# huggingface/parler-tts

Hardware: NVIDIA H100
Metric: audio codec tokens/sec (all codebooks) (higher is better)
Workload: dtype bf16

## Files before the change

include/ptts_b200.h:

```cpp
#ifndef PTTS_B200_H
#define PTTS_B200_H

#include <stdint.h>

#ifdef __cplusplus
extern "C" {
#endif

#define PTTS_OK 0
#define PTTS_EINVAL 1
#define PTTS_ECUDA 2
#define PTTS_ESTATE 3

#define PTTS_BF16 0
#define PTTS_F32 1
#define PTTS_I64 2
#define PTTS_I32 3

#define PTTS_HEAD_DIM 64

typedef struct ptts_decoder_config {
  int32_t hidden_size;
  int32_t num_layers;
  int32_t num_heads;
// ... 190 lines not shown

int ptts_dac_blob_bytes(const ptts_dac_config* cfg, int64_t* out_bytes);
int ptts_dac_num_tensors(const ptts_dac_config* cfg, int32_t* out);
int ptts_dac_pack(const ptts_dac_config* cfg, void* blob, int32_t name_id, const void* src,
                  int32_t src_dtype, int64_t numel, void* stream);
int ptts_dac_workspace_bytes(const ptts_dac_config* cfg, int32_t B, int32_t T, int64_t* out_bytes);
int ptts_dac_decode(const ptts_dac_config* cfg, const void* blob, void* workspace, int64_t workspace_bytes,
                    const int64_t* codes, int32_t B, int32_t T, void* audio_out, void* stream);
int ptts_dac_decode2(const ptts_dac_config* cfg, const void* blob, void* workspace, int64_t workspace_bytes,
                     const int64_t* codes, int32_t B, int32_t T, const int32_t* frame_lengths, void* audio_out,
                     void* stream);
int ptts_dac_decode3(const ptts_dac_config* cfg, const void* blob, void* workspace, int64_t workspace_bytes,
                     const int64_t* codes, int32_t B, int32_t T_codes, int32_t T,
                     const int32_t* frame_start, const int32_t* frame_lengths,
                     const int32_t* emit_lo, const int32_t* emit_hi, void* audio_out, void* stream);

int ptts_dac_encoder_blob_bytes(const ptts_dac_config* cfg, int64_t* out_bytes);
int ptts_dac_encoder_num_tensors(const ptts_dac_config* cfg, int32_t* out);
int ptts_dac_encoder_pack(const ptts_dac_config* cfg, void* enc_blob, int32_t name_id, const void* src,
                          int32_t src_dtype, int64_t numel, void* stream);
int ptts_dac_encode_workspace_bytes(const ptts_dac_config* cfg, int32_t B, int32_t samples, int64_t* out_bytes);
int ptts_dac_encode(const ptts_dac_config* cfg, const void* dec_blob, const void* enc_blob, void* workspace,
                    int64_t workspace_bytes, const void* audio, int32_t B, int32_t samples, int32_t n_q, int64_t* codes_out,
                    void* latents_out, void* stream);
int ptts_dac_encode2(const ptts_dac_config* cfg, const void* dec_blob, const void* enc_blob, void* workspace,
                     int64_t workspace_bytes, const void* audio, int32_t B, int32_t samples, const int32_t* sample_lengths,
                     int32_t n_q, int64_t* codes_out, void* latents_out, void* stream);

int ptts_op_dac_conv(int32_t dtype, int32_t kernel, int32_t kind, int32_t B, int32_t Cin, int32_t Cout, int32_t T, int32_t taps,
                     int32_t dil_or_stride, int32_t samples, const void* weight, const void* bias, const void* alpha,
                     const void* alpha_next, const void* x, const void* res, void* out_raw, void* out_act, int32_t tanh_out,
                     const int32_t* frame_lengths, int32_t frames, void* scratch, void* stream);

#ifdef __cplusplus
}
#endif
#endif
```

parler_tts_b200/_lib.py:

```python
from __future__ import annotations
import ctypes as C
import os

import torch

_HERE = os.path.dirname(os.path.abspath(__file__))
LIB_PATH = os.environ.get("PTTS_LIB") or os.path.join(_HERE, "csrc", "libptts_b200.so")

BF16, F32, I64, I32 = 0, 1, 2, 3
OK, EINVAL, ECUDA, ESTATE = 0, 1, 2, 3


class DecoderConfigC(C.Structure):
    _fields_ = [(n, C.c_int32) for n in (
        "hidden_size", "num_layers", "num_heads", "num_kv_heads", "num_cross_kv_heads", "ffn_dim", "vocab_size",
        "num_codebooks", "max_positions", "rope", "activation", "dtype", "bos_token_id", "pad_token_id",
        "eos_token_id")] + [("rope_theta", C.c_float), ("layer_norm_eps", C.c_float)]


class GenParamsC(C.Structure):
    _fields_ = [("max_length", C.c_int32), ("min_new_tokens", C.c_int32), ("do_sample", C.c_int32),
                ("top_k", C.c_int32), ("top_p", C.c_float), ("temperature", C.c_float), ("seed", C.c_uint64),
                ("suppress_special", C.c_int32), ("codebook_size", C.c_int32),
                ("row_base", C.c_int32), ("input_len", C.c_int32)]
# ... 61 lines not shown
    "ptts_session_logits": (C.c_int, [_VP, C.POINTER(_VP)]),
    "ptts_session_scores": (C.c_int, [_VP, C.POINTER(_VP)]),
    "ptts_session_raw_ids": (C.c_int, [_VP, C.POINTER(_VP), C.POINTER(_I32)]),
    "ptts_session_state": (C.c_int, [_VP, C.POINTER(_VP)]),
    "ptts_session_eos_seen": (C.c_int, [_VP, C.POINTER(_VP)]),
    "ptts_session_launches": (C.c_int, [_VP, C.POINTER(_I64)]),
    "ptts_session_fused": (C.c_int, [_VP, C.POINTER(_I32)]),
    "ptts_session_set_profile": (C.c_int, [_VP, _VP]),
    "ptts_delay_build": (C.c_int, [_VP, _I32, _I32, _I32, _I64, _I64, _I32, _VP, _VP]),
    "ptts_delay_apply": (C.c_int, [_VP, _I32, _I32, _I64, _VP, _I64, _VP, _VP]),
    "ptts_logits_processor": (C.c_int, [_VP, _I32, _I32, _I64, _VP, _I32, _I64, _I32, _VP, _VP]),
    "ptts_op_sample_phase": (C.c_int, [_VP, _I32, _VP]),
    "ptts_op_linear": (C.c_int, [C.POINTER(DecoderConfigC), _VP, _I32, _I32, _VP, _I32, _I32, _I32, _VP, _VP, _VP]),
    "ptts_op_linear2": (C.c_int, [C.POINTER(DecoderConfigC), _VP, _I32, _I32, _VP, _I32, _I32, _I32, _VP, _VP, _I32, _VP, _VP]),
    "ptts_op_attention": (C.c_int, [_I32, _I32, _I32, _I32, _I32, _I32, _I32, _I32, _I32, _I32, _VP, _VP, _VP, _VP, _VP, _VP,
                                    _I32, _I32, _VP, _VP]),
    "ptts_op_attention_probs": (C.c_int, [_I32, _I32, _I32, _I32, _I32, _I32, _I32, _I32, _I32, _I32, _VP, _VP, _VP, _I64, _VP,
                                          _VP, _I32, _VP, _VP]),
    "ptts_dac_blob_bytes": (C.c_int, [C.POINTER(DacConfigC), C.POINTER(_I64)]),
    "ptts_dac_num_tensors": (C.c_int, [C.POINTER(DacConfigC), C.POINTER(_I32)]),
    "ptts_dac_pack": (C.c_int, [C.POINTER(DacConfigC), _VP, _I32, _VP, _I32, _I64, _VP]),
    "ptts_dac_workspace_bytes": (C.c_int, [C.POINTER(DacConfigC), _I32, _I32, C.POINTER(_I64)]),
    "ptts_dac_decode": (C.c_int, [C.POINTER(DacConfigC), _VP, _VP, _I64, _VP, _I32, _I32, _VP, _VP]),
    "ptts_dac_decode2": (C.c_int, [C.POINTER(DacConfigC), _VP, _VP, _I64, _VP, _I32, _I32, _VP, _VP, _VP]),
    "ptts_dac_decode3": (C.c_int, [C.POINTER(DacConfigC), _VP, _VP, _I64, _VP, _I32, _I32, _I32, _VP, _VP, _VP, _VP, _VP, _VP]),
    "ptts_dac_encoder_blob_bytes": (C.c_int, [C.POINTER(DacConfigC), C.POINTER(_I64)]),
    "ptts_dac_encoder_num_tensors": (C.c_int, [C.POINTER(DacConfigC), C.POINTER(_I32)]),
    "ptts_dac_encoder_pack": (C.c_int, [C.POINTER(DacConfigC), _VP, _I32, _VP, _I32, _I64, _VP]),
    "ptts_dac_encode_workspace_bytes": (C.c_int, [C.POINTER(DacConfigC), _I32, _I32, C.POINTER(_I64)]),
    "ptts_dac_encode": (C.c_int, [C.POINTER(DacConfigC), _VP, _VP, _VP, _I64, _VP, _I32, _I32, _I32, _VP, _VP, _VP]),
    "ptts_dac_encode2": (C.c_int, [C.POINTER(DacConfigC), _VP, _VP, _VP, _I64, _VP, _I32, _I32, _VP, _I32, _VP, _VP, _VP]),
    "ptts_op_dac_conv": (C.c_int, [_I32, _I32, _I32, _I32, _I32, _I32, _I32, _I32, _I32, _I32, _VP, _VP, _VP, _VP, _VP, _VP, _VP,
                                   _VP, _I32, _VP, _I32, _VP, _VP]),
}
EXPORTED_SYMBOLS = tuple(_SIGS)

_lib = None


def lib():
    global _lib
    if _lib is None:
        if not os.path.exists(LIB_PATH):
            raise ImportError(
                f"{LIB_PATH} is missing: build it with `python parler_tts_b200/csrc/build.py` "
                "(or __graft_entry__.build()).  parler_tts_b200 has no CPU / PyTorch fallback.")
        l = C.CDLL(LIB_PATH)
        for name, (res, args) in _SIGS.items():
            fn = getattr(l, name)
            fn.restype, fn.argtypes = res, args
        _lib = l
    return _lib


def check(code: int):
    if code == OK:
        return
    msg = lib().ptts_last_error().decode("utf-8", "replace")
    if code == EINVAL:
        raise ValueError(msg)
    raise RuntimeError(msg)


def dtype_code(dt: torch.dtype) -> int:
    if dt == torch.bfloat16:
        return BF16
# ... 22 lines not shown
```

parler_tts_b200/csrc/api.cu:

```cuda
#include <cstdarg>
#include <cstdlib>
#include <cstring>
#include <new>
#include <vector>

#include "common.cuh"
#include "dac.h"
#include "kernels.h"
#include "layout.h"
#include "step.h"

namespace ptts {
static thread_local std::string g_err;
void set_error(const std::string& m) { g_err = m; }
int fail(int code, const char* fmt, ...) {
  char buf[1024];
  va_list ap;
  va_start(ap, fmt);
  vsnprintf(buf, sizeof(buf), fmt, ap);
  va_end(ap);
  g_err = buf;
  return code;
}
static bool env_flag(const char* name, bool dflt) {
// ... 1212 lines not shown
        a.alpha = tiled;
      }
      a.out = out_raw; a.tanh_out = tanh_out ? 1 : 0;
      return launch_conv(a, dtype, B, st, ragged(a));
    }
    case 1: {
      PTTS_REQUIRE(conv_tc_supported(a.Cin, a.Cout), "op_dac_conv: conv_tc_kernel does not take Cin %d, Cout %d", a.Cin, a.Cout);
      PTTS_REQUIRE(!alpha && !tanh_out && samples == 0, "op_dac_conv: conv_tc_kernel has no input snake, tanh or samples");
      PTTS_REQUIRE(!out_act == !alpha_next, "op_dac_conv: out_act and alpha_next go together");
      if (kind == 2) {
        if (int e = pack_strided_conv(weight, dtype, scratch, PTTS_BF16, Cout, Cin, s, 1, st)) return e;
      } else if (int e = pack_conv_kmajor(weight, dtype, scratch, kind == 1 ? Cin : Cout, kind == 1 ? Cout : Cin, k_src, kind == 1, st)) {
        return e;
      }
      return launch_conv_tc(a, scratch, a.n_taps * a.n_phase, alpha_next, out_raw, out_act, B, st, ragged(a));
    }
    case 2: {
      PTTS_REQUIRE(kind == 0 && Cout == 1 && taps == 7 && dil_or_stride == 1 && final_conv_supported(Cin),
                   "op_dac_conv: the final conv is conv_same(C, 1, T, 7, 1) with final_conv_supported(C), got Cin %d Cout %d taps %d", Cin, Cout, taps);
      PTTS_REQUIRE(!alpha && !alpha_next && !res && !out_act && out_raw && tanh_out && samples == 0, "op_dac_conv: the final conv writes tanh to out_raw only");
      if (int e = pack_conv(weight, dtype, scratch, dtype, Cout, Cin, 7, 0, st)) return e;
      return launch_final_conv_tanh(x, scratch, bias, out_raw, Cin, T, B, frame_lengths, frames, st);
    }
    default: {
      PTTS_REQUIRE(kind == 0 && Cin == 1 && taps == 7 && dil_or_stride == 1 && samples > 0 && samples <= T,
                   "op_dac_conv: the input conv is conv_same(1, C, T, 7, 1) over 1..T samples");
      PTTS_REQUIRE(!alpha && !res && !tanh_out && !frame_lengths && alpha_next && out_raw && out_act, "op_dac_conv: the input conv writes raw and snake_{alpha_next}");
      if (int e = pack_conv(weight, dtype, scratch, dtype, Cout, 1, 7, 0, st)) return e;
      return launch_enc_input_conv(x, scratch, bias, alpha_next, out_raw, out_act, Cout, samples, T, B, nullptr, 0, st);
    }
  }
}

}
```

parler_tts_b200/csrc/attention.cu:

```cuda
#include "common.cuh"
#include "kernels.h"
#include "attn_core.cuh"

namespace ptts {

template <typename T>
__global__ void __launch_bounds__(ATT_THREADS) attention_kernel(AttnArgs p) {
  extern __shared__ __align__(16) float sm[];
  pdl_launch_dependents();
  pdl_wait();
  if (p.ctrl != nullptr && p.ctrl->active == 0) return;
  const int per = (p.q_len + (int)gridDim.z - 1) / (int)gridDim.z;
  attention_item<T>(p, blockIdx.y, blockIdx.x, sm, threadIdx.x, [] { __syncthreads(); }, (int)blockIdx.z * per, (int)(blockIdx.z + 1) * per);
}

template <typename T, bool RAGGED>
__global__ void __launch_bounds__(256) attention_decode_kernel(AttnArgs p) {
  extern __shared__ __align__(128) unsigned char smd[];
  const int warp = threadIdx.x >> 5, lane = threadIdx.x & 31;
  uint64_t* bars = reinterpret_cast<uint64_t*>(smd) + 2 * warp;
  unsigned char* sm_warp = smd + 128 + (size_t)warp * attn_decode_smem_per_warp<T>();
  attention_decode_init_warp(bars, lane);
  pdl_launch_dependents();
  pdl_wait();
  if (p.ctrl != nullptr && p.ctrl->active == 0) return;
  const int pair = warp >> 1, part = warp & 1;
  const int it = blockIdx.x * 4 + pair;
  if (it >= p.B * p.nkv) return;
  int past = p.past_len;
  if (p.past_from_ctrl) past = p.prefix + p.ctrl->cur_len - 1 - (RAGGED ? row_shift(p.shift, it / p.nkv) : 0);
  uint32_t parity = 0;
  float* xch = reinterpret_cast<float*>(smd + 128 + (size_t)8 * attn_decode_smem_per_warp<T>()) + pair * 128;
  attention_decode_item_warp<T>(p, it / p.nkv, it % p.nkv, past, sm_warp, bars, lane, parity, part, 2, xch, pair + 1);
}

constexpr int PRE_TC_WARPS = 8;
constexpr int PRE_TC_WARP_BYTES = 2 * ATT_TC_STAGE_BYTES + 768;
__global__ void __launch_bounds__(PRE_TC_WARPS * 32) attention_prefill_tc_kernel(AttnArgs p) {
  extern __shared__ __align__(128) unsigned char smp[];
  const int warp = threadIdx.x >> 5, lane = threadIdx.x & 31;
  uint64_t* bars = reinterpret_cast<uint64_t*>(smp) + 2 * warp;
  unsigned char* ring0 = smp + 128 + (size_t)warp * PRE_TC_WARP_BYTES;
  unsigned char* ring1 = ring0 + ATT_TC_STAGE_BYTES;
  float* fbuf = reinterpret_cast<float*>(ring1 + ATT_TC_STAGE_BYTES);
  attention_decode_init_warp(bars, lane);
  pdl_launch_dependents();
  pdl_wait();
  if (p.ctrl != nullptr && p.ctrl->active == 0) return;
  const int b = blockIdx.y, h = blockIdx.x;
  const int past = p.past_len;
  const int kvb = b / p.kv_b_div;
  bf16* kc = reinterpret_cast<bf16*>(p.kcache) + (size_t)kvb * p.kv_b_stride + (size_t)h * p.kv_h_stride;
  bf16* vc = reinterpret_cast<bf16*>(p.vcache) + (size_t)kvb * p.kv_b_stride + (size_t)h * p.kv_h_stride;
  if (!p.cross) {
    const bf16* rope_cos = reinterpret_cast<const bf16*>(p.rope_cos);
    const bf16* rope_sin = reinterpret_cast<const bf16*>(p.rope_sin);
    for (int idx = threadIdx.x; idx < p.q_len * 2 * HD; idx += PRE_TC_WARPS * 32) {
      const int j = idx / (2 * HD), e = idx - j * 2 * HD, d = e & (HD - 1);
      const size_t r = (size_t)b * p.q_len + j;
      const int pos = past + j;
      if (e < HD) {
        const bf16* src = reinterpret_cast<const bf16*>(p.knew) + r * p.ldkv + p.k_col0 + h * HD;
        float x = __bfloat162float(src[d]);
        if (p.rope) {
          const float xp = __bfloat162float(src[d < HD / 2 ? d + HD / 2 : d - HD / 2]);
          x = rope_elem<bf16>(x, xp, d, rope_cos + (size_t)pos * HD, rope_sin + (size_t)pos * HD);
        }
        kc[(size_t)pos * HD + kv_swz(pos, d)] = __float2bfloat16_rn(x);
      } else {
        const bf16* src = reinterpret_cast<const bf16*>(p.vnew) + r * p.ldkv + p.v_col0 + h * HD;
        vc[(size_t)pos * HD + kv_swz(pos, d)] = src[d];
      }
    }
    __threadfence();
    asm volatile("fence.proxy.async.global;" ::: "memory");
    __syncthreads();
  }
  uint32_t parity = 0;
  for (int j = warp; j < p.q_len; j += PRE_TC_WARPS) {
    const size_t r = (size_t)b * p.q_len + j;
    TcItem it{};
    it.q = reinterpret_cast<const bf16*>(p.q) + r * p.ldq + p.q_col0 + (size_t)h * HD;
    it.knew = nullptr; it.vnew = nullptr;
    it.kc = kc; it.vc = vc;
    it.km = p.key_mask ? p.key_mask + (size_t)kvb * p.mask_ld : nullptr; it.mask_len = p.mask_len;
    it.n_cached = p.cross ? p.kv_len : past + j + 1;
    it.pos = past + j; it.cross = 1;
    it.rope = p.rope; it.rope_cos = reinterpret_cast<const bf16*>(p.rope_cos); it.rope_sin = reinterpret_cast<const bf16*>(p.rope_sin);
    it.scale = p.scale;
    it.out = reinterpret_cast<bf16*>(p.out) + r * p.ldo + (size_t)h * HD;
    attention_decode_item_warp_tc(it, ring0, ring1, fbuf, bars, lane, parity, 0, 1, nullptr, 0);
    asm volatile("fence.proxy.async.shared::cta;" ::: "memory");
    __syncwarp();
  }
}

int launch_attention(const AttnArgs& a, int dtype, cudaStream_t st, bool pdl, bool prefill_tc) {
  if (a.q_len > 1 && dtype == PTTS_BF16 && a.nh == a.nkv && a.kv_t_stride == HD && !a.past_from_ctrl && prefill_tc) {
    const size_t smem = 128 + (size_t)PRE_TC_WARPS * PRE_TC_WARP_BYTES;
    static bool attr_p = false;
    if (!attr_p) {
      PTTS_CHECK_CUDA(cudaFuncSetAttribute(attention_prefill_tc_kernel, cudaFuncAttributeMaxDynamicSharedMemorySize, (int)smem));
      attr_p = true;
    }
    cudaLaunchConfig_t cfg{};
    cfg.gridDim = dim3(a.nkv, a.B);
    cfg.blockDim = dim3(PRE_TC_WARPS * 32);
    cfg.dynamicSmemBytes = smem;
    cfg.stream = st;
    cudaLaunchAttribute at[1];
    at[0].id = cudaLaunchAttributeProgrammaticStreamSerialization;
    at[0].val.programmaticStreamSerializationAllowed = 1;
    cfg.attrs = at;
    cfg.numAttrs = pdl ? 1 : 0;
    PTTS_CHECK_CUDA(cudaLaunchKernelEx(&cfg, attention_prefill_tc_kernel, a));
    return PTTS_OK;
  }
  if (a.q_len == 1) {
    const size_t smem_d = 128 + (size_t)8 * (dtype == PTTS_BF16 ? attn_decode_smem_per_warp<bf16>() : attn_decode_smem_per_warp<float>()) + 4 * 128 * sizeof(float);
    static bool attr_d = false;
    if (!attr_d) {
      PTTS_CHECK_CUDA(cudaFuncSetAttribute(attention_decode_kernel<bf16, false>, cudaFuncAttributeMaxDynamicSharedMemorySize, 200 * 1024));
      PTTS_CHECK_CUDA(cudaFuncSetAttribute(attention_decode_kernel<float, false>, cudaFuncAttributeMaxDynamicSharedMemorySize, 200 * 1024));
      PTTS_CHECK_CUDA(cudaFuncSetAttribute(attention_decode_kernel<bf16, true>, cudaFuncAttributeMaxDynamicSharedMemorySize, 200 * 1024));
      PTTS_CHECK_CUDA(cudaFuncSetAttribute(attention_decode_kernel<float, true>, cudaFuncAttributeMaxDynamicSharedMemorySize, 200 * 1024));
      attr_d = true;
    }
    cudaLaunchConfig_t cfg{};
    cfg.gridDim = dim3((a.B * a.nkv + 3) / 4);
    cfg.blockDim = dim3(256);
    cfg.dynamicSmemBytes = smem_d;
    cfg.stream = st;
    cudaLaunchAttribute at[1];
    at[0].id = cudaLaunchAttributeProgrammaticStreamSerialization;
    at[0].val.programmaticStreamSerializationAllowed = 1;
    cfg.attrs = at;
    cfg.numAttrs = pdl ? 1 : 0;
    const bool rg = a.shift != nullptr;
    if (dtype == PTTS_BF16) PTTS_CHECK_CUDA(cudaLaunchKernelEx(&cfg, rg ? attention_decode_kernel<bf16, true> : attention_decode_kernel<bf16, false>, a));
    else PTTS_CHECK_CUDA(cudaLaunchKernelEx(&cfg, rg ? attention_decode_kernel<float, true> : attention_decode_kernel<float, false>, a));
    return PTTS_OK;
  }
  const int kv_capacity = a.kv_capacity;
  PTTS_REQUIRE(a.B > 0 && a.nkv > 0 && a.q_len > 0, "attention: empty problem");
  const size_t smem = (size_t)(HD + ATT_WARPS * HD + 8 + kv_capacity) * sizeof(float);
  PTTS_REQUIRE(smem <= 200 * 1024, "attention: kv length %d needs %zu B of shared memory (> 200 KB)", kv_capacity, smem);
  static bool attr_done = false;
// ... 24 lines not shown
```

parler_tts_b200/csrc/dac.cu:

```cuda
#include <utility>
#include <vector>

#include "common.cuh"
#include "dac.h"

namespace ptts {

template <typename T>
__device__ __forceinline__ float snake_fn(float x, float alpha, float inv) {
  const float s = DT<T>::rnd(sinf(DT<T>::rnd(alpha * x)));
  return DT<T>::rnd(x + DT<T>::rnd(inv * DT<T>::rnd(s * s)));
}

constexpr int CT_M = 64, CT_N = 64, CT_K = 16, CT_AROWS = 128, CT_MAXTAPS = 7;

template <typename T, bool SAMPLES, bool WINDOW = false>
__global__ void __launch_bounds__(256) conv_kernel(ConvArgs p, RowLengths rl) {
  __shared__ float As[CT_K][CT_AROWS];
  __shared__ __align__(16) float Bs[CT_MAXTAPS][CT_K][CT_N];
  const int tid = threadIdx.x, tx = tid & 15, ty = tid >> 4;
  const int phase = blockIdx.z % p.n_phase, b = blockIdx.z / p.n_phase;
  const int q0 = blockIdx.x * CT_M, co0 = blockIdx.y * CT_N;
  const int wt_base = p.wt_base + phase * p.wt_phase_step;
  const int off_last = p.off_base + (p.n_taps - 1) * p.off_step;
// ... 267 lines not shown
  const DacWindow* win;
  std::vector<Margin> m;
  size_t i = 1;
  RowLengths next(int up_in, int up_out) {
    RowLengths r{fl, T, up_in, up_out};
    if (win != nullptr) { r.emit_lo = win->emit_lo; r.emit_hi = win->emit_hi; r.m_lo = m[i].lo; r.m_hi = m[i].hi; }
    i++;
    return r;
  }
};

static int decode_tc(const ptts_dac_config& c, const DacLayout& L, const char* bl, const DacWorkspace& W, void* ws, int B, int T,
                     WalkRows& rows, void* audio, cudaStream_t st) {
  auto P = [&](int i) { return (const void*)(bl + L.t[i].off); };
  auto conv = [&](ConvArgs a, const void* x, int w, int b, const void* res, void* out_raw, void* out_act, const void* alpha_next) {
    a.x = x; a.bias = P(b); a.res = res;
    return launch_conv_tc(a, bl + L.t[w].off_k, a.n_taps * a.n_phase, alpha_next, out_raw, out_act, B, st, rows.next(a.Tin / T, a.Tout / T));
  };
  char* act = W.buf(ws, 0);
  char* oth = W.buf(ws, 1);
  char* res = W.buf(ws, 2);
  const int C = c.decoder_dim, nb = c.n_blocks;
  if (int e = conv(conv_same(c.latent_dim, C, T, 7, 1), W.buf(ws, 3), L.conv1_w, L.conv1_b, nullptr, nullptr, act, P(L.block[0].snake1))) return e;
  int Tl = T;
  for (int bi = 0; bi < nb; bi++) {
    const DacDecBlock& blk = L.block[bi];
    const int cout = C >> (bi + 1), s = c.strides[bi];
    if (int e = conv(conv_up(C >> bi, cout, Tl, s), act, blk.conv_t1_w, blk.conv_t1_b, nullptr, res, oth, P(blk.res[0].snake1))) return e;
    std::swap(act, oth);
    Tl *= s;
    for (int r = 0; r < 3; r++) {
      const DacResUnit& u = blk.res[r];
      const int next = r < 2 ? blk.res[r + 1].snake1 : bi + 1 < nb ? L.block[bi + 1].snake1 : L.snake1;
      if (int e = conv(conv_same(cout, cout, Tl, 7, kDilation[r]), act, u.conv1_w, u.conv1_b, nullptr, nullptr, oth, P(u.snake2))) return e;
      if (int e = conv(conv_same(cout, cout, Tl, 1, 1), oth, u.conv2_w, u.conv2_b, res, res, act, P(next))) return e;
    }
  }
  const int cl = C >> nb;
  const RowLengths rl = rows.next(Tl / T, Tl / T);
  if (final_conv_supported(cl))
    return launch_final_conv_tanh(act, P(L.conv2_w), P(L.conv2_b), audio, cl, Tl, B, rl.frame_lengths, T, st, rl.emit_lo, rl.emit_hi);
  ConvArgs f = conv_same(cl, 1, Tl, 7, 1);
  f.x = act; f.w = P(L.conv2_w); f.bias = P(L.conv2_b); f.out = audio; f.tanh_out = 1;
  return launch_conv(f, c.dtype, B, st, rl);
}

static int decode_generic(const ptts_dac_config& c, const DacLayout& L, const char* bl, const DacWorkspace& W, void* ws, int B, int T,
                          WalkRows& rows, void* audio, cudaStream_t st) {
  auto P = [&](int i) { return (const void*)(bl + L.t[i].off); };
  auto conv = [&](ConvArgs a, const void* x, const void* alpha, int w, int b, const void* res, void* out) {
    a.x = x; a.alpha = alpha; a.w = P(w); a.bias = P(b); a.res = res; a.out = out;
    return launch_conv(a, c.dtype, B, st, rows.next(a.Tin / T, a.Tout / T));
  };
  char* cur = W.buf(ws, 0);
  char* oth = W.buf(ws, 1);
  const int C = c.decoder_dim;
  if (int e = conv(conv_same(c.latent_dim, C, T, 7, 1), W.buf(ws, 3), nullptr, L.conv1_w, L.conv1_b, nullptr, cur)) return e;
  int Tl = T;
  for (int bi = 0; bi < c.n_blocks; bi++) {
    const DacDecBlock& blk = L.block[bi];
    const int cout = C >> (bi + 1), s = c.strides[bi];
    if (int e = conv(conv_up(C >> bi, cout, Tl, s), cur, P(blk.snake1), blk.conv_t1_w, blk.conv_t1_b, nullptr, oth)) return e;
    std::swap(cur, oth);
    Tl *= s;
    for (int r = 0; r < 3; r++) {
      const DacResUnit& u = blk.res[r];
// ... 42 lines not shown
```

parler_tts_b200/csrc/dac.h:

```cpp
#pragma once
#include <vector>
#include "common.cuh"
#include "layout.h"

namespace ptts {

struct ConvArgs {
  const void* x; const void* w; const void* bias; const void* alpha; const void* res; void* out;
  int Cin, Cout, Tin, Tout, q_count;
  int n_taps, off_base, off_step, wt_base, wt_step;
  int n_phase, wt_phase_step, o_mul, o_add, o_phase_step;
  int tanh_out;
};
static inline ConvArgs conv_same(int Cin, int Cout, int T, int taps, int dil) {
  ConvArgs a{};
  a.Cin = Cin; a.Cout = Cout; a.Tin = T; a.Tout = T; a.q_count = T;
  a.n_taps = taps; a.off_base = -((taps - 1) / 2) * dil; a.off_step = dil; a.wt_base = 0; a.wt_step = 1;
  a.n_phase = 1; a.wt_phase_step = 0; a.o_mul = 1; a.o_add = 0; a.o_phase_step = 0;
  return a;
}
static inline ConvArgs conv_up(int Cin, int Cout, int T, int s) {
  ConvArgs a{};
  a.Cin = Cin; a.Cout = Cout; a.Tin = T; a.Tout = T * s; a.q_count = T + 1;
  a.n_taps = 2; a.off_base = 0; a.off_step = -1; a.wt_base = 0; a.wt_step = s;
// ... 13 lines not shown

__device__ __forceinline__ int row_frames(const int32_t* frame_lengths, int b, int frames) {
  return min(max(__ldg(frame_lengths + b), 0), frames);
}
__device__ __forceinline__ int row_samples(const int32_t* sample_lengths, int b, int samples) {
  return min(max(__ldg(sample_lengths + b), 1), samples);
}
template <bool SAMPLES>
__device__ __forceinline__ int row_frames(const int32_t* lengths, int b, int frames, int hop) {
  if constexpr (SAMPLES) return (row_samples(lengths, b, frames * hop) + hop - 1) / hop;
  else return row_frames(lengths, b, frames);
}
__device__ __forceinline__ int2 needed_rows(const int32_t* emit_lo, const int32_t* emit_hi, int b, int n, int up_out, int m_lo, int m_hi) {
  const int lo = min(max(__ldg(emit_lo + b), 0), n), hi = min(max(__ldg(emit_hi + b), lo), n);
  if (lo == hi) return make_int2(0, 0);
  return make_int2(lo * up_out - m_lo, hi * up_out + m_hi);
}

struct FromCodesArgs {
  const int64_t* codes;
  const void* codebooks; const void* proj_w; const void* proj_b;
  void* z;
  int K, D, C, T, codebook_size;
  const int32_t* frame_lengths;
  const int32_t* frame_start; const int32_t* emit_lo; const int32_t* emit_hi;
  int codes_T, m_lo, m_hi;
};
int launch_from_codes(const FromCodesArgs& a, int dtype, int B, cudaStream_t st);
int pack_conv(const void* src, int src_dtype, void* dst, int dst_dtype, int d0, int d1, int k, int transposed, cudaStream_t st);
bool conv_tc_supported(int Cin, int Cout);
int launch_conv_tc(const ConvArgs& a, const void* w_kmajor, int taps_total, const void* alpha_next, void* out_raw, void* out_act, int B, cudaStream_t st,
                   const RowLengths& rl = RowLengths{});
int pack_conv_kmajor(const void* src, int src_dtype, void* dst, int d0, int d1, int k, int transposed, cudaStream_t st);
bool final_conv_supported(int C);
int launch_final_conv_tanh(const void* x, const void* w, const void* bias, void* out, int C, int T, int B, const int32_t* frame_lengths,
                           int frames, cudaStream_t st, const int32_t* emit_lo = nullptr, const int32_t* emit_hi = nullptr);

enum { DK_PLAIN = 0, DK_CONV = 1, DK_CONVT = 2 };
struct DacTensor {
  int kind;
  int d0, d1, k;
  int64_t off;
  int64_t numel;
  int64_t off_k;
};

struct DacResUnit { int snake1, conv1_w, conv1_b, snake2, conv2_w, conv2_b; };
struct DacDecBlock { int snake1, conv_t1_w, conv_t1_b; DacResUnit res[3]; };
struct DacEncBlock { DacResUnit res[3]; int snake1, conv1_w, conv1_b; };

struct DacLayout {
  std::vector<DacTensor> t;
  int64_t codebooks, proj_w, proj_b;
  int conv1_w, conv1_b;
  DacDecBlock block[8];
  int snake1, conv2_w, conv2_b;
  int64_t total;
  int es;
};

static inline int validate_dac(const ptts_dac_config& c) {
  PTTS_REQUIRE(c.dtype == PTTS_BF16 || c.dtype == PTTS_F32, "dac dtype must be bf16 or f32");
  PTTS_REQUIRE(c.n_blocks >= 1 && c.n_blocks <= 8, "dac n_blocks out of range");
  PTTS_REQUIRE(c.n_codebooks >= 1 && c.n_codebooks <= 32 && c.codebook_dim >= 1 && c.codebook_dim <= 16 &&
               c.n_codebooks * c.codebook_dim <= 256, "dac codebook shape unsupported");
  PTTS_REQUIRE((c.decoder_dim >> c.n_blocks) >= 1, "dac decoder_dim too small for n_blocks");
// ... 190 lines not shown
```

parler_tts_b200/csrc/dac_tc.cu:

```cuda
#include <algorithm>
#include <type_traits>
#include <mutex>
#include <vector>

#include "common.cuh"
#include "dac.h"
#include "wgmma.cuh"

namespace ptts {

constexpr int TC_M = wg::M_TILE;
constexpr int TC_K = wg::K_STAGE;

struct ConvTcArgs {
  int Cin, Cout, Tin, Tout, q_count;
  int n_taps, off_base, off_step, wt_base, wt_step;
  int n_phase, wt_phase_step, o_mul, o_add, o_phase_step;
  const bf16* bias;
  const bf16* res;
  bf16* out_raw;
  bf16* out_act;
  const bf16* alpha_next;
  const int32_t* frame_lengths;
  int frames, up_in, up_out, hop;
// ... 62 lines not shown
      }
    }
    return;
  }

  const __nv_bfloat162* bias2 = reinterpret_cast<const __nv_bfloat162*>(chan);
  const __nv_bfloat162* alpha2 = reinterpret_cast<const __nv_bfloat162*>(chan + NT);
  const __nv_bfloat162* inv2 = reinterpret_cast<const __nv_bfloat162*>(chan + 2 * NT);
  const int qrow = q0 + 64 * (threadIdx.x >> 7);
#pragma unroll
  for (int h = 0; h < 2; h++) {
    const int q = qrow + wg::frag_row(2 * h);
    const int to = q * p.o_mul + p.o_add + phase * p.o_phase_step;
    if (q >= p.q_count || to < 0 || to >= to_end) continue;
    const size_t orow = ((size_t)b * p.Tout + to) * p.Cout + n0;
#pragma unroll
    for (int j = 0; j < NT / 8; j++) {
      const int i = 4 * j + 2 * h, c = wg::frag_col(i);
      const float2 bb = __bfloat1622float2(bias2[c >> 1]);
      __nv_bfloat162 r2 = __floats2bfloat162_rn(acc[i] + bb.x, acc[i + 1] + bb.y);
      if (p.res != nullptr) r2 = __hadd2(*reinterpret_cast<const __nv_bfloat162*>(p.res + orow + c), r2);
      if (p.out_raw != nullptr) *reinterpret_cast<__nv_bfloat162*>(p.out_raw + orow + c) = r2;
      if (p.out_act != nullptr) {
        const __nv_bfloat162 ax = __hmul2(alpha2[c >> 1], r2);
        const float2 axf = __bfloat1622float2(ax);
        const __nv_bfloat162 sn = __floats2bfloat162_rn(__sinf(axf.x), __sinf(axf.y));
        const __nv_bfloat162 sq = __hmul2(sn, sn);
        *reinterpret_cast<__nv_bfloat162*>(p.out_act + orow + c) = __hadd2(r2, __hmul2_rn(inv2[c >> 1], sq));
      }
    }
  }
}

typedef CUresult (*EncodeTiledFn)(CUtensorMap*, CUtensorMapDataType, cuuint32_t, void*, const cuuint64_t*, const cuuint64_t*, const cuuint32_t*,
                                  const cuuint32_t*, CUtensorMapInterleave, CUtensorMapSwizzle, CUtensorMapL2promotion, CUtensorMapFloatOOBfill);
static EncodeTiledFn encode_fn() {
  static EncodeTiledFn fn = nullptr;
  if (!fn) {
    void* p = nullptr;
    cudaDriverEntryPointQueryResult q;
    if (cudaGetDriverEntryPoint("cuTensorMapEncodeTiled", &p, cudaEnableDefault, &q) == cudaSuccess && q == cudaDriverEntryPointSuccess) fn = (EncodeTiledFn)p;
  }
  return fn;
}
static int encode_map(CUtensorMap* m, const void* base, uint64_t d0, uint64_t d1, uint64_t d2, uint32_t box1);

struct MapKey { const void* base; uint64_t d0, d1, d2; uint32_t box1; };
struct MapEntry { MapKey k; CUtensorMap m; };
static int make_map(CUtensorMap* m, const void* base, uint64_t d0, uint64_t d1, uint64_t d2, uint32_t box1) {
  static std::mutex mu;
  static std::vector<MapEntry> cache;
  std::lock_guard<std::mutex> lock(mu);
  for (const MapEntry& e : cache)
    if (e.k.base == base && e.k.d0 == d0 && e.k.d1 == d1 && e.k.d2 == d2 && e.k.box1 == box1) { *m = e.m; return PTTS_OK; }
  if (int e = encode_map(m, base, d0, d1, d2, box1)) return e;
  if (cache.size() >= 4096) cache.clear();
  cache.push_back(MapEntry{MapKey{base, d0, d1, d2, box1}, *m});
  return PTTS_OK;
}
static int encode_map(CUtensorMap* m, const void* base, uint64_t d0, uint64_t d1, uint64_t d2, uint32_t box1) {
  EncodeTiledFn fn = encode_fn();
  if (!fn) return fail(PTTS_ECUDA, "cuTensorMapEncodeTiled is not available from the driver");
  cuuint64_t dims[3] = {d0, d1, d2};
  cuuint64_t strides[2] = {d0 * 2, d0 * d1 * 2};
  cuuint32_t box[3] = {(cuuint32_t)TC_K, box1, 1};
  cuuint32_t es[3] = {1, 1, 1};
// ... 33 lines not shown
  return p.frame_lengths != nullptr && p.hop > 0 ? launch_conv_tile_t<NT, true>(mx, mw, q, B, st) : launch_conv_tile_t<NT, false>(mx, mw, q, B, st);
}

int launch_conv_tc(const ConvArgs& a, const void* w_kmajor, int taps_total, const void* alpha_next, void* out_raw, void* out_act, int B, cudaStream_t st,
                   const RowLengths& rl) {
  ConvTcWindowArgs p{};
  p.Cin = a.Cin; p.Cout = a.Cout; p.Tin = a.Tin; p.Tout = a.Tout; p.q_count = a.q_count;
  p.n_taps = a.n_taps; p.off_base = a.off_base; p.off_step = a.off_step; p.wt_base = a.wt_base; p.wt_step = a.wt_step;
  p.n_phase = a.n_phase; p.wt_phase_step = a.wt_phase_step; p.o_mul = a.o_mul; p.o_add = a.o_add; p.o_phase_step = a.o_phase_step;
  const int n_tile = conv_tc_ntile(a.Cout);
  p.bias = (const bf16*)a.bias; p.res = (const bf16*)a.res; p.out_raw = (bf16*)out_raw; p.out_act = (bf16*)out_act; p.alpha_next = (const bf16*)alpha_next;
  p.frame_lengths = rl.frame_lengths; p.frames = rl.frames; p.up_in = rl.up_in; p.up_out = rl.up_out; p.hop = rl.hop;
  p.emit_lo = rl.emit_lo; p.emit_hi = rl.emit_hi; p.m_lo = rl.m_lo; p.m_hi = rl.m_hi;
  if (rl.emit_lo != nullptr) {
    PTTS_REQUIRE(rl.frame_lengths != nullptr && rl.hop == 0 && rl.emit_hi != nullptr, "conv_tc: a windowed decode needs frame lengths");
    PTTS_REQUIRE(rl.m_hi <= TC_M, "conv_tc: window margin %d rows is wider than the %d-row zero band", rl.m_hi, TC_M);
  }
  if (rl.frame_lengths != nullptr) {
    const int reach = std::max(std::max(a.off_base, a.off_base + (a.n_taps - 1) * a.off_step), 0) + (a.q_count - a.Tin);
    PTTS_REQUIRE(reach <= TC_M, "conv_tc: a ragged batch reads %d rows past a row's end, more than the %d-row zero band", reach, TC_M);
    PTTS_REQUIRE(rl.frames > 0 && a.Tin == rl.frames * rl.up_in && a.Tout == rl.frames * rl.up_out, "conv_tc: ragged lengths do not match the shape");
  }
  CUtensorMap mx, mw;
  if (int e = make_map(&mx, a.x, (uint64_t)a.Cin, (uint64_t)a.Tin, (uint64_t)B, TC_M)) return e;
  if (int e = make_map(&mw, w_kmajor, (uint64_t)a.Cin, (uint64_t)a.Cout, (uint64_t)taps_total, (uint32_t)n_tile)) return e;
  switch (n_tile) {
    case 128: return launch_conv_tile<128>(mx, mw, p, B, st);
    case 96: return launch_conv_tile<96>(mx, mw, p, B, st);
    case 64: return launch_conv_tile<64>(mx, mw, p, B, st);
    default: return launch_conv_tile<32>(mx, mw, p, B, st);
  }
}

template <typename S>
__global__ void pack_conv_kmajor_kernel(const S* src, bf16* dst, int d0, int d1, int k, int transposed) {
  const int64_t i = (int64_t)blockIdx.x * blockDim.x + threadIdx.x;
  const int64_t n = (int64_t)d0 * d1 * k;
  if (i >= n) return;
  const int kk = (int)(i % k);
  const int b1 = (int)((i / k) % d1), b0 = (int)(i / ((int64_t)k * d1));
  const int ci = transposed ? b0 : b1, co = transposed ? b1 : b0;
  const int Cin = transposed ? d0 : d1, Cout = transposed ? d1 : d0;
  float v;
  if constexpr (sizeof(S) == 2) v = __bfloat162float(src[i]); else v = src[i];
  dst[((size_t)kk * Cout + co) * Cin + ci] = __float2bfloat16_rn(v);
}
int pack_conv_kmajor(const void* src, int src_dtype, void* dst, int d0, int d1, int k, int transposed, cudaStream_t st) {
  const int64_t n = (int64_t)d0 * d1 * k;
  const int blocks = (int)((n + 255) / 256);
  if (src_dtype == PTTS_BF16) pack_conv_kmajor_kernel<bf16><<<blocks, 256, 0, st>>>((const bf16*)src, (bf16*)dst, d0, d1, k, transposed);
  else pack_conv_kmajor_kernel<float><<<blocks, 256, 0, st>>>((const float*)src, (bf16*)dst, d0, d1, k, transposed);
  PTTS_LAUNCH_CHECK();
  return PTTS_OK;
}

}
```

Baseline: 255,000.

## Fuse DAC residual unit convs into one wgmma kernel; split prefill KV append

Adds a fused tensor-core kernel for the DAC residual unit. It runs the dilated 7-tap conv and the snake activation, writes the activated tile back into shared memory, then runs the 1x1 conv with the residual add and the next snake, all in one launch. This removes the intermediate global round trip and one kernel launch per residual unit when C is 96 or 192. Separately, attention prefill moves the KV-cache append and rope into its own kernel, halves the warps per block and spreads query rows over a third grid dimension for more parallelism. The cost is an extra launch per self-attention prefill and much larger, more complex fused kernel code.

Measured after the change: 255,700, median of 6. No clear change (+0.3%).

```diff
diff --git a/include/ptts_b200.h b/include/ptts_b200.h
--- a/include/ptts_b200.h
+++ b/include/ptts_b200.h
@@ -246,6 +246,10 @@
                      const void* alpha_next, const void* x, const void* res, void* out_raw, void* out_act, int32_t tanh_out,
                      const int32_t* frame_lengths, int32_t frames, void* scratch, void* stream);
 
+int ptts_op_dac_res_unit(int32_t B, int32_t C, int32_t T, int32_t dil, const void* w7, const void* b7, const void* alpha2, const void* w1,
+                         const void* b1, const void* alpha_next, const void* x, void* res, void* out_act, const int32_t* frame_lengths,
+                         int32_t frames, const int32_t* emit_lo, const int32_t* emit_hi, int32_t m_lo, int32_t m_hi, void* scratch, void* stream);
+
 #ifdef __cplusplus
 }
 #endif
diff --git a/parler_tts_b200/_lib.py b/parler_tts_b200/_lib.py
--- a/parler_tts_b200/_lib.py
+++ b/parler_tts_b200/_lib.py
@@ -117,6 +117,8 @@
     "ptts_dac_encode2": (C.c_int, [C.POINTER(DacConfigC), _VP, _VP, _VP, _I64, _VP, _I32, _I32, _VP, _I32, _VP, _VP, _VP]),
     "ptts_op_dac_conv": (C.c_int, [_I32, _I32, _I32, _I32, _I32, _I32, _I32, _I32, _I32, _I32, _VP, _VP, _VP, _VP, _VP, _VP, _VP,
                                    _VP, _I32, _VP, _I32, _VP, _VP]),
+    "ptts_op_dac_res_unit": (C.c_int, [_I32, _I32, _I32, _I32, _VP, _VP, _VP, _VP, _VP, _VP, _VP, _VP, _VP, _VP, _I32, _VP, _VP,
+                                       _I32, _I32, _VP, _VP]),
 }
 EXPORTED_SYMBOLS = tuple(_SIGS)
 
diff --git a/parler_tts_b200/csrc/api.cu b/parler_tts_b200/csrc/api.cu
--- a/parler_tts_b200/csrc/api.cu
+++ b/parler_tts_b200/csrc/api.cu
@@ -1268,4 +1268,28 @@
   }
 }
 
-}
+int ptts_op_dac_res_unit(int32_t B, int32_t C, int32_t T, int32_t dil, const void* w7, const void* b7, const void* alpha2, const void* w1,
+                         const void* b1, const void* alpha_next, const void* x, void* res, void* out_act, const int32_t* frame_lengths,
+                         int32_t frames, const int32_t* emit_lo, const int32_t* emit_hi, int32_t m_lo, int32_t m_hi, void* scratch, void* stream) {
+  PTTS_REQUIRE(w7 && b7 && alpha2 && w1 && b1 && alpha_next && x && res && out_act && scratch, "null argument");
+  PTTS_REQUIRE(B > 0 && T > 0, "op_dac_res_unit: bad shape B=%d T=%d", B, T);
+  PTTS_REQUIRE(res_unit_tc_supported(C), "op_dac_res_unit: C %d is not 96 or 192", C);
+  PTTS_REQUIRE(dil >= 1 && 3 * dil <= 128, "op_dac_res_unit: dilation %d outside 1..42", dil);
+  PTTS_REQUIRE(x != out_act && res != out_act && res != x, "op_dac_res_unit: x, res and out_act must be three buffers");
+  PTTS_REQUIRE(frame_lengths == nullptr || (frames > 0 && T % frames == 0), "op_dac_res_unit: %d rows are not whole frames of %d", T, frames);
+  PTTS_REQUIRE(emit_lo == nullptr || (frame_lengths != nullptr && emit_hi != nullptr && m_lo >= 0 && m_hi >= 0),
+               "op_dac_res_unit: a window needs frame lengths, emit_hi and margins >= 0");
+  cudaStream_t st = (cudaStream_t)stream;
+  char* w7k = (char*)scratch;
+  char* w1k = w7k + align_up((int64_t)7 * C * C * 2, 1024);
+  if (int e = pack_conv_kmajor(w7, PTTS_BF16, w7k, C, C, 7, 0, st)) return e;
+  if (int e = pack_conv_kmajor(w1, PTTS_BF16, w1k, C, C, 1, 0, st)) return e;
+  RowLengths rl1{};
+  if (frame_lengths != nullptr) rl1 = RowLengths{frame_lengths, frames, T / frames, T / frames, 0, emit_lo, emit_hi, m_lo, m_hi};
+  RowLengths rl7 = rl1;
+  rl7.m_lo += 3 * dil; rl7.m_hi += 3 * dil;
+  const ResUnitTc u{C, T, dil, x, w7k, b7, alpha2, w1k, b1, alpha_next, res, out_act};
+  return launch_res_unit_tc(u, B, st, rl7, rl1);
+}
+
+}
diff --git a/parler_tts_b200/csrc/attention.cu b/parler_tts_b200/csrc/attention.cu
--- a/parler_tts_b200/csrc/attention.cu
+++ b/parler_tts_b200/csrc/attention.cu
@@ -34,8 +34,40 @@
   attention_decode_item_warp<T>(p, it / p.nkv, it % p.nkv, past, sm_warp, bars, lane, parity, part, 2, xch, pair + 1);
 }
 
-constexpr int PRE_TC_WARPS = 8;
+constexpr int PRE_TC_WARPS = 4;
 constexpr int PRE_TC_WARP_BYTES = 2 * ATT_TC_STAGE_BYTES + 768;
+__global__ void __launch_bounds__(PRE_TC_WARPS * 32) prefill_kv_append_kernel(AttnArgs p) {
+  pdl_launch_dependents();
+  pdl_wait();
+  if (p.ctrl != nullptr && p.ctrl->active == 0) return;
+  const int b = blockIdx.y, h = blockIdx.x;
+  const int past = p.past_len;
+  const int kvb = b / p.kv_b_div;
+  bf16* kc = reinterpret_cast<bf16*>(p.kcache) + (size_t)kvb * p.kv_b_stride + (size_t)h * p.kv_h_stride;
+  bf16* vc = reinterpret_cast<bf16*>(p.vcache) + (size_t)kvb * p.kv_b_stride + (size_t)h * p.kv_h_stride;
+  const bf16* rope_cos = reinterpret_cast<const bf16*>(p.rope_cos);
+  const bf16* rope_sin = reinterpret_cast<const bf16*>(p.rope_sin);
+  for (int idx = threadIdx.x; idx < p.q_len * 2 * HD; idx += PRE_TC_WARPS * 32) {
+    const int j = idx / (2 * HD), e = idx - j * 2 * HD, d = e & (HD - 1);
+    const size_t r = (size_t)b * p.q_len + j;
+    const int pos = past + j;
+    if (e < HD) {
+      const bf16* src = reinterpret_cast<const bf16*>(p.knew) + r * p.ldkv + p.k_col0 + h * HD;
+      float x = __bfloat162float(src[d]);
+      if (p.rope) {
+        const float xp = __bfloat162float(src[d < HD / 2 ? d + HD / 2 : d - HD / 2]);
+        x = rope_elem<bf16>(x, xp, d, rope_cos + (size_t)pos * HD, rope_sin + (size_t)pos * HD);
+      }
+      kc[(size_t)pos * HD + kv_swz(pos, d)] = __float2bfloat16_rn(x);
+    } else {
+      const bf16* src = reinterpret_cast<const bf16*>(p.vnew) + r * p.ldkv + p.v_col0 + h * HD;
+      vc[(size_t)pos * HD + kv_swz(pos, d)] = src[d];
+    }
+  }
+  __threadfence();
+  asm volatile("fence.proxy.async.global;" ::: "memory");
+}
+
 __global__ void __launch_bounds__(PRE_TC_WARPS * 32) attention_prefill_tc_kernel(AttnArgs p) {
   extern __shared__ __align__(128) unsigned char smp[];
   const int warp = threadIdx.x >> 5, lane = threadIdx.x & 31;
@@ -52,32 +84,9 @@
   const int kvb = b / p.kv_b_div;
   bf16* kc = reinterpret_cast<bf16*>(p.kcache) + (size_t)kvb * p.kv_b_stride + (size_t)h * p.kv_h_stride;
   bf16* vc = reinterpret_cast<bf16*>(p.vcache) + (size_t)kvb * p.kv_b_stride + (size_t)h * p.kv_h_stride;
-  if (!p.cross) {
-    const bf16* rope_cos = reinterpret_cast<const bf16*>(p.rope_cos);
-    const bf16* rope_sin = reinterpret_cast<const bf16*>(p.rope_sin);
-    for (int idx = threadIdx.x; idx < p.q_len * 2 * HD; idx += PRE_TC_WARPS * 32) {
-      const int j = idx / (2 * HD), e = idx - j * 2 * HD, d = e & (HD - 1);
-      const size_t r = (size_t)b * p.q_len + j;
-      const int pos = past + j;
-      if (e < HD) {
-        const bf16* src = reinterpret_cast<const bf16*>(p.knew) + r * p.ldkv + p.k_col0 + h * HD;
-        float x = __bfloat162float(src[d]);
-        if (p.rope) {
-          const float xp = __bfloat162float(src[d < HD / 2 ? d + HD / 2 : d - HD / 2]);
-          x = rope_elem<bf16>(x, xp, d, rope_cos + (size_t)pos * HD, rope_sin + (size_t)pos * HD);
-        }
-        kc[(size_t)pos * HD + kv_swz(pos, d)] = __float2bfloat16_rn(x);
-      } else {
-        const bf16* src = reinterpret_cast<const bf16*>(p.vnew) + r * p.ldkv + p.v_col0 + h * HD;
-        vc[(size_t)pos * HD + kv_swz(pos, d)] = src[d];
-      }
-    }
-    __threadfence();
-    asm volatile("fence.proxy.async.global;" ::: "memory");
-    __syncthreads();
-  }
+  const int j0 = (int)blockIdx.z * PRE_TC_WARPS, j1 = min(j0 + PRE_TC_WARPS, p.q_len);
   uint32_t parity = 0;
-  for (int j = warp; j < p.q_len; j += PRE_TC_WARPS) {
+  for (int j = j0 + warp; j < j1; j += PRE_TC_WARPS) {
     const size_t r = (size_t)b * p.q_len + j;
     TcItem it{};
     it.q = reinterpret_cast<const bf16*>(p.q) + r * p.ldq + p.q_col0 + (size_t)h * HD;
@@ -104,7 +113,7 @@
       attr_p = true;
     }
     cudaLaunchConfig_t cfg{};
-    cfg.gridDim = dim3(a.nkv, a.B);
+    cfg.gridDim = dim3(a.nkv, a.B, (a.q_len + PRE_TC_WARPS - 1) / PRE_TC_WARPS);
     cfg.blockDim = dim3(PRE_TC_WARPS * 32);
     cfg.dynamicSmemBytes = smem;
     cfg.stream = st;
@@ -113,6 +122,13 @@
     at[0].val.programmaticStreamSerializationAllowed = 1;
     cfg.attrs = at;
     cfg.numAttrs = pdl ? 1 : 0;
+    if (!a.cross) {
+      cudaLaunchConfig_t ca = cfg;
+      ca.gridDim = dim3(a.nkv, a.B);
+      ca.dynamicSmemBytes = 0;
+      PTTS_CHECK_CUDA(cudaLaunchKernelEx(&ca, prefill_kv_append_kernel, a));
+      cfg.numAttrs = 1;
+    }
     PTTS_CHECK_CUDA(cudaLaunchKernelEx(&cfg, attention_prefill_tc_kernel, a));
     return PTTS_OK;
   }
diff --git a/parler_tts_b200/csrc/dac.cu b/parler_tts_b200/csrc/dac.cu
--- a/parler_tts_b200/csrc/dac.cu
+++ b/parler_tts_b200/csrc/dac.cu
@@ -323,6 +323,14 @@
     for (int r = 0; r < 3; r++) {
       const DacResUnit& u = blk.res[r];
       const int next = r < 2 ? blk.res[r + 1].snake1 : bi + 1 < nb ? L.block[bi + 1].snake1 : L.snake1;
+      if (res_unit_tc_supported(cout)) {
+        const ResUnitTc ru{cout, Tl, kDilation[r], act, bl + L.t[u.conv1_w].off_k, P(u.conv1_b), P(u.snake2),
+                           bl + L.t[u.conv2_w].off_k, P(u.conv2_b), P(next), res, oth};
+        const RowLengths rl7 = rows.next(Tl / T, Tl / T);
+        if (int e = launch_res_unit_tc(ru, B, st, rl7, rows.next(Tl / T, Tl / T))) return e;
+        std::swap(act, oth);
+        continue;
+      }
       if (int e = conv(conv_same(cout, cout, Tl, 7, kDilation[r]), act, u.conv1_w, u.conv1_b, nullptr, nullptr, oth, P(u.snake2))) return e;
       if (int e = conv(conv_same(cout, cout, Tl, 1, 1), oth, u.conv2_w, u.conv2_b, res, res, act, P(next))) return e;
     }
diff --git a/parler_tts_b200/csrc/dac.h b/parler_tts_b200/csrc/dac.h
--- a/parler_tts_b200/csrc/dac.h
+++ b/parler_tts_b200/csrc/dac.h
@@ -69,6 +69,14 @@
 int launch_conv_tc(const ConvArgs& a, const void* w_kmajor, int taps_total, const void* alpha_next, void* out_raw, void* out_act, int B, cudaStream_t st,
                    const RowLengths& rl = RowLengths{});
 int pack_conv_kmajor(const void* src, int src_dtype, void* dst, int d0, int d1, int k, int transposed, cudaStream_t st);
+bool res_unit_tc_supported(int C);
+struct ResUnitTc {
+  int C, T, dil;
+  const void* x; const void* w7_kmajor; const void* bias7; const void* alpha2;
+  const void* w1_kmajor; const void* bias1; const void* alpha_next;
+  void* res; void* out_act;
+};
+int launch_res_unit_tc(const ResUnitTc& u, int B, cudaStream_t st, const RowLengths& rl7 = RowLengths{}, const RowLengths& rl1 = RowLengths{});
 bool final_conv_supported(int C);
 int launch_final_conv_tanh(const void* x, const void* w, const void* bias, void* out, int C, int T, int B, const int32_t* frame_lengths,
                            int frames, cudaStream_t st, const int32_t* emit_lo = nullptr, const int32_t* emit_hi = nullptr);
diff --git a/parler_tts_b200/csrc/dac_tc.cu b/parler_tts_b200/csrc/dac_tc.cu
--- a/parler_tts_b200/csrc/dac_tc.cu
+++ b/parler_tts_b200/csrc/dac_tc.cu
@@ -118,6 +118,180 @@
   }
 }
 
+constexpr int RU_NT = 96;
+struct ResUnitTcArgs {
+  int T, dil;
+  const bf16* bias7; const bf16* alpha2;
+  const bf16* bias1; const bf16* alpha_next;
+  bf16* res;
+  bf16* out_act;
+  const int32_t* frame_lengths;
+  int frames, up;
+  const int32_t* emit_lo; const int32_t* emit_hi;
+  int m_lo, m_hi;
+};
+template <int C> constexpr int RU_CHUNKS = (C + TC_K - 1) / TC_K;
+template <int C> constexpr size_t res_unit_smem_bytes() { return wg::smem_bytes<C>(6 * C * (int)sizeof(bf16)); }
+static_assert(RU_CHUNKS<192> <= wg::STAGES && RU_CHUNKS<96> <= wg::STAGES, "res_unit: the k1 operand needs one stage per 64-channel chunk");
+static_assert((RU_NT * TC_K * 2) % 1024 == 0, "res_unit: each 96-column half of a B slot starts on a swizzle atom");
+static_assert(res_unit_smem_bytes<96>() <= 227 * 1024 / 2, "res_unit<96>: two CTAs per SM");
+static_assert(res_unit_smem_bytes<192>() <= 227 * 1024, "res_unit<192>: one CTA per SM");
+
+template <int C>
+__global__ void __launch_bounds__(wg::THREADS, C <= RU_NT ? 2 : 1)
+res_unit_tc_kernel(const __grid_constant__ CUtensorMap map_x, const __grid_constant__ CUtensorMap map_w7,
+                   const __grid_constant__ CUtensorMap map_w1, const ResUnitTcArgs p) {
+  static_assert(C % RU_NT == 0 && C <= 2 * RU_NT, "res_unit: C is 96 or 192");
+  constexpr int NH = C / RU_NT, KC = RU_CHUNKS<C>, N7 = 7 * KC, N1 = KC, STAGE = wg::STAGE_BYTES<C>;
+  extern __shared__ unsigned char smem_raw[];
+  const wg::Pipe pipe = wg::pipe_setup<C>(smem_raw);
+  bf16* chan = reinterpret_cast<bf16*>(pipe.extra);
+  const int b = blockIdx.y, q0 = blockIdx.x * TC_M, T = p.T;
+  bool compute = true;
+  if (p.frame_lengths != nullptr) {
+    const int q_end = row_frames(p.frame_lengths, b, p.frames) * p.up;
+    if ((int)blockIdx.x > q_end / TC_M + 1) return;
+    if (q0 >= q_end) compute = false;
+  }
+  if (p.emit_lo != nullptr) {
+    const int2 need = needed_rows(p.emit_lo, p.emit_hi, b, row_frames(p.frame_lengths, b, p.frames), p.up, p.m_lo, p.m_hi);
+    if (q0 + TC_M - 1 < need.x || q0 >= need.y) return;
+  }
+  const int to_end = p.frame_lengths != nullptr ? row_frames(p.frame_lengths, b, p.frames) * p.up : T;
+
+  if (threadIdx.x == 0) {
+    asm volatile("prefetch.tensormap [%0];" ::"l"(&map_x) : "memory");
+    asm volatile("prefetch.tensormap [%0];" ::"l"(&map_w7) : "memory");
+    asm volatile("prefetch.tensormap [%0];" ::"l"(&map_w1) : "memory");
+  }
+  for (int c = threadIdx.x; c < C; c += blockDim.x) {
+    chan[c] = p.bias7[c];
+    chan[3 * C + c] = p.bias1[c];
+    const bf16 a2 = p.alpha2[c], an = p.alpha_next[c];
+    chan[C + c] = a2;
+    chan[2 * C + c] = __float2bfloat16_rn(1.0f / __bfloat162float(__float2bfloat16_rn(__bfloat162float(a2) + 1e-9f)));
+    chan[4 * C + c] = an;
+    chan[5 * C + c] = __float2bfloat16_rn(1.0f / __bfloat162float(__float2bfloat16_rn(__bfloat162float(an) + 1e-9f)));
+  }
+  __syncthreads();
+
+  const int warp = threadIdx.x >> 5, lane = threadIdx.x & 31;
+  if (warp == wg::PRODUCER_WARP) {
+    if (lane == 0 && compute) {
+      for (int it = 0; it < N7 + N1; it++) {
+        const int s = it % wg::STAGES, use = it / wg::STAGES;
+        if (use > 0) wg::mbar_wait(&pipe.empty[s], (use - 1) & 1);
+        unsigned char* a_dst = pipe.stages + (size_t)s * STAGE;
+        if (it < N7) {
+          const int j = it / KC, kc = it - j * KC;
+          mbar_expect_tx(&pipe.full[s], (uint32_t)(wg::A_BYTES + C * TC_K * 2));
+          wg::tma_load_3d(a_dst, &map_x, kc * TC_K, q0 + (j - 3) * p.dil, b, &pipe.full[s]);
+          wg::tma_load_3d(a_dst + wg::A_BYTES, &map_w7, kc * TC_K, 0, j, &pipe.full[s]);
+        } else {
+          mbar_expect_tx(&pipe.full[s], (uint32_t)(C * TC_K * 2));
+          wg::tma_load_3d(a_dst + wg::A_BYTES, &map_w1, (it - N7) * TC_K, 0, 0, &pipe.full[s]);
+        }
+      }
+    }
+    if (to_end < T) {
+      for (int e = lane; e < TC_M * (C / 8); e += 32) {
+        const int q = q0 + e / (C / 8), c = 8 * (e % (C / 8));
+        if (q >= T || q < to_end) continue;
+        const size_t o = ((size_t)b * T + q) * C + c;
+        *reinterpret_cast<uint4*>(p.res + o) = make_uint4(0u, 0u, 0u, 0u);
+        *reinterpret_cast<uint4*>(p.out_act + o) = make_uint4(0u, 0u, 0u, 0u);
+      }
+    }
+    return;
+  }
+  if (!compute) return;
+
+  const int wgi = warp >> 2;
+  const uint32_t a_row0 = (uint32_t)wgi * 64 * 128;
+  float acc[NH][RU_NT / 2];
+#pragma unroll
+  for (int h = 0; h < NH; h++)
+#pragma unroll
+    for (int i = 0; i < RU_NT / 2; i++) acc[h][i] = 0.f;
+  const __nv_bfloat162* chan2 = reinterpret_cast<const __nv_bfloat162*>(chan);
+  for (int it = 0; it < N7 + N1; it++) {
+    const int s = it % wg::STAGES;
+    if (it == N7) {
+      asm volatile("wgmma.wait_group.sync.aligned 0;" ::: "memory");
+      if (lane == 0) wg::mbar_arrive(&pipe.empty[(N7 - 1) % wg::STAGES]);
+#pragma unroll
+      for (int hr = 0; hr < 2; hr++) {
+        const int r = 64 * wgi + wg::frag_row(2 * hr), q = q0 + r;
+        const bool keep = q < T && q < to_end;
+#pragma unroll
+        for (int h = 0; h < NH; h++)
+#pragma unroll
+          for (int j = 0; j < RU_NT / 8; j++) {
+            const int i = 4 * j + 2 * hr, c = RU_NT * h + wg::frag_col(i);
+            __nv_bfloat162 v = __floats2bfloat162_rn(0.f, 0.f);
+            if (keep) {
+              const float2 bb = __bfloat1622float2(chan2[c >> 1]);
+              const __nv_bfloat162 r2 = __floats2bfloat162_rn(acc[h][i] + bb.x, acc[h][i + 1] + bb.y);
+              const __nv_bfloat162 ax = __hmul2(chan2[C / 2 + (c >> 1)], r2);
+              const float2 axf = __bfloat1622float2(ax);
+              const __nv_bfloat162 sn = __floats2bfloat162_rn(__sinf(axf.x), __sinf(axf.y));
+              const __nv_bfloat162 sq = __hmul2(sn, sn);
+              v = __hadd2(r2, __hmul2_rn(chan2[C + (c >> 1)], sq));
+            }
+            unsigned char* slot = pipe.stages + (size_t)((N7 + c / TC_K) % wg::STAGES) * STAGE;
+            *reinterpret_cast<__nv_bfloat162*>(slot + r * 128 + ((((c % TC_K) >> 3) ^ (r & 7)) << 4) + (c & 7) * 2) = v;
+          }
+      }
+      if constexpr (C % TC_K != 0) {
+        unsigned char* slot = pipe.stages + (size_t)((N7 + KC - 1) % wg::STAGES) * STAGE;
+        constexpr int V0 = (C % TC_K) / 8, NV = 8 - V0;
+        for (int e = threadIdx.x & 127; e < 64 * NV; e += 128) {
+          const int r = 64 * wgi + e / NV, v16 = V0 + e % NV;
+          *reinterpret_cast<uint4*>(slot + r * 128 + ((v16 ^ (r & 7)) << 4)) = make_uint4(0u, 0u, 0u, 0u);
+        }
+      }
+      asm volatile("fence.proxy.async.shared::cta;" ::: "memory");
+      asm volatile("bar.sync %0, 128;" ::"r"(1 + wgi) : "memory");
+    }
+    wg::mbar_wait(&pipe.full[s], (it / wg::STAGES) & 1);
+    const uint32_t a_addr = smem_u32(pipe.stages + (size_t)s * STAGE);
+    const uint64_t da = wg::desc_sw128(a_addr + a_row0), db = wg::desc_sw128(a_addr + wg::A_BYTES);
+    const int first = it == 0 || it == N7;
+    asm volatile("wgmma.fence.sync.aligned;" ::: "memory");
+#pragma unroll
+    for (int k = 0; k < TC_K / 16; k++)
+#pragma unroll
+      for (int h = 0; h < NH; h++)
+        wg::mma<RU_NT>(acc[h], da + (uint64_t)(2 * k), db + (uint64_t)(h * (RU_NT * 128 / 16) + 2 * k), (first && k == 0) ? 0 : 1);
+    asm volatile("wgmma.commit_group.sync.aligned;" ::: "memory");
+    asm volatile("wgmma.wait_group.sync.aligned 1;" ::: "memory");
+    if (it > 0 && it != N7 && lane == 0) wg::mbar_arrive(&pipe.empty[(it - 1) % wg::STAGES]);
+  }
+  asm volatile("wgmma.wait_group.sync.aligned 0;" ::: "memory");
+
+#pragma unroll
+  for (int hr = 0; hr < 2; hr++) {
+    const int q = q0 + 64 * wgi + wg::frag_row(2 * hr);
+    if (q >= T || q >= to_end) continue;
+    const size_t orow = ((size_t)b * T + q) * C;
+#pragma unroll
+    for (int h = 0; h < NH; h++)
+#pragma unroll
+      for (int j = 0; j < RU_NT / 8; j++) {
+        const int i = 4 * j + 2 * hr, c = RU_NT * h + wg::frag_col(i);
+        const float2 bb = __bfloat1622float2(chan2[3 * C / 2 + (c >> 1)]);
+        __nv_bfloat162 r2 = __floats2bfloat162_rn(acc[h][i] + bb.x, acc[h][i + 1] + bb.y);
+        r2 = __hadd2(*reinterpret_cast<const __nv_bfloat162*>(p.res + orow + c), r2);
+        *reinterpret_cast<__nv_bfloat162*>(p.res + orow + c) = r2;
+        const __nv_bfloat162 ax = __hmul2(chan2[2 * C + (c >> 1)], r2);
+        const float2 axf = __bfloat1622float2(ax);
+        const __nv_bfloat162 sn = __floats2bfloat162_rn(__sinf(axf.x), __sinf(axf.y));
+        const __nv_bfloat162 sq = __hmul2(sn, sn);
+        *reinterpret_cast<__nv_bfloat162*>(p.out_act + orow + c) = __hadd2(r2, __hmul2_rn(chan2[5 * C / 2 + (c >> 1)], sq));
+      }
+  }
+}
+
 typedef CUresult (*EncodeTiledFn)(CUtensorMap*, CUtensorMapDataType, cuuint32_t, void*, const cuuint64_t*, const cuuint64_t*, const cuuint32_t*,
                                   const cuuint32_t*, CUtensorMapInterleave, CUtensorMapSwizzle, CUtensorMapL2promotion, CUtensorMapFloatOOBfill);
 static EncodeTiledFn encode_fn() {
@@ -217,6 +391,48 @@
   }
 }
 
+bool res_unit_tc_supported(int C) { return C == RU_NT || C == 2 * RU_NT; }
+
+template <int C>
+static int launch_res_unit_t(const CUtensorMap& mx, const CUtensorMap& m7, const CUtensorMap& m1, const ResUnitTcArgs& p, int B, cudaStream_t st) {
+  constexpr size_t smem = res_unit_smem_bytes<C>();
+  static bool attr = false;
+  if (!attr) {
+    PTTS_CHECK_CUDA(cudaFuncSetAttribute(res_unit_tc_kernel<C>, cudaFuncAttributeMaxDynamicSharedMemorySize, (int)smem));
+    attr = true;
+  }
+  res_unit_tc_kernel<C><<<dim3((p.T + TC_M - 1) / TC_M, B), wg::THREADS, smem, st>>>(mx, m7, m1, p);
+  PTTS_LAUNCH_CHECK();
+  return PTTS_OK;
+}
+
+int launch_res_unit_tc(const ResUnitTc& u, int B, cudaStream_t st, const RowLengths& rl7, const RowLengths& rl1) {
+  const int C = u.C, T = u.T;
+  PTTS_REQUIRE(res_unit_tc_supported(C), "res_unit_tc: C %d is not 96 or 192", C);
+  PTTS_REQUIRE(T > 0 && u.dil >= 1 && 3 * u.dil <= TC_M, "res_unit_tc: T %d, dilation %d", T, u.dil);
+  PTTS_REQUIRE(u.x != u.out_act && u.res != u.out_act && u.res != u.x, "res_unit_tc: x, res and out_act must be three buffers");
+  PTTS_REQUIRE(rl7.frame_lengths == rl1.frame_lengths && rl7.frames == rl1.frames && rl7.emit_lo == rl1.emit_lo && rl7.hop == 0 && rl1.hop == 0,
+               "res_unit_tc: the two layers' row lengths differ");
+  ResUnitTcArgs p{};
+  p.T = T; p.dil = u.dil;
+  p.bias7 = (const bf16*)u.bias7; p.alpha2 = (const bf16*)u.alpha2; p.bias1 = (const bf16*)u.bias1; p.alpha_next = (const bf16*)u.alpha_next;
+  p.res = (bf16*)u.res; p.out_act = (bf16*)u.out_act;
+  p.frame_lengths = rl1.frame_lengths; p.frames = rl1.frames; p.up = rl1.frame_lengths != nullptr ? rl1.up_out : 0;
+  p.emit_lo = rl1.emit_lo; p.emit_hi = rl1.emit_hi; p.m_lo = rl1.m_lo; p.m_hi = rl1.m_hi;
+  if (rl1.frame_lengths != nullptr)
+    PTTS_REQUIRE(rl1.frames > 0 && rl1.up_in == rl1.up_out && T == rl1.frames * rl1.up_out && rl7.up_in == rl1.up_in && rl7.up_out == rl1.up_out,
+                 "res_unit_tc: ragged lengths do not match the shape");
+  if (rl1.emit_lo != nullptr) {
+    PTTS_REQUIRE(rl1.frame_lengths != nullptr && rl1.emit_hi != nullptr, "res_unit_tc: a windowed decode needs frame lengths");
+    PTTS_REQUIRE(rl7.m_hi <= TC_M && rl1.m_hi <= rl7.m_hi && rl1.m_lo <= rl7.m_lo, "res_unit_tc: window margins %d / %d", rl7.m_hi, rl1.m_hi);
+  }
+  CUtensorMap mx, m7, m1;
+  if (int e = make_map(&mx, u.x, (uint64_t)C, (uint64_t)T, (uint64_t)B, TC_M)) return e;
+  if (int e = make_map(&m7, u.w7_kmajor, (uint64_t)C, (uint64_t)C, 7, (uint32_t)C)) return e;
+  if (int e = make_map(&m1, u.w1_kmajor, (uint64_t)C, (uint64_t)C, 1, (uint32_t)C)) return e;
+  return C == RU_NT ? launch_res_unit_t<RU_NT>(mx, m7, m1, p, B, st) : launch_res_unit_t<2 * RU_NT>(mx, m7, m1, p, B, st);
+}
+
 template <typename S>
 __global__ void pack_conv_kmajor_kernel(const S* src, bf16* dst, int d0, int d1, int k, int transposed) {
   const int64_t i = (int64_t)blockIdx.x * blockDim.x + threadIdx.x;
```
